# qfall/tools

Hardware: NVIDIA B200
Metric: samp_p_preimages_per_s (higher is better)
Workload: dtype f64

## Files before the change

### tools_b200/csrc/api.cu

```cuda
#include <algorithm>
#include <cmath>
#include <cstdio>
#include <cstring>
#include <string>
#include <vector>

#include "../../include/qfall_b200.h"
#include "common.cuh"
#include "kernels.h"

namespace {

typedef unsigned __int128 u128;
typedef __int128 i128;

struct Dev {
    void* p = nullptr;
    size_t cap = 0;
    cudaError_t ensure(size_t bytes) {
        if (bytes <= cap) return cudaSuccess;
        if (p) cudaFree(p);
        p = nullptr;
        cap = 0;
        cudaError_t e = cudaMalloc(&p, bytes);
// ... 715 lines not shown
        g.B = Bc; g.N = (int)ctx->m_bar; g.K = (int)ctx->nk;
        g.out_kind = 2; g.sign = 1; g.q = 0; g.base = nullptr; g.ldbase = 0; g.out = P; g.ldout = ldm;
        g.flag = ctx->dFlag.as<int>();
        LAUNCH(ctx_gemm_i8(ctx, g));
    } else {
        LAUNCH(ctx_gemm(ctx, Z, ldnk, ctx->dR.as<double>(), ldnk, P, ldm, Bc, (int)ctx->m_bar, (int)ctx->nk, 1.0, 1.0, 0));
    }
    LAUNCH(qf_launch_finalize_pert(P, ldm, Z, ldnk, dE, ctx->m, Bc, (int)ctx->m, (int)ctx->m_bar, ctx->dFlag.as<int>(),
                                   ctx->stream));
    return QF_OK;
}

qf_status samp_p_pert_chunk(qf_ctx* ctx, const int64_t* dUin, int Bc, uint64_t seed, uint64_t first, int32_t* dE,
                            const int32_t* dTidx = nullptr) {
    QF_TRY(pert_perturbation(ctx, Bc, seed, first));
    QF_TRY(pert_ap(ctx, dUin, Bc, ctx->w[4].as<int64_t>()));
    return pert_finish(ctx, Bc, seed, first, dE, dTidx);
}

constexpr long NP_SIZES[4] = {64, 256, 1024, 4096};
constexpr int NP_TOP = 4;
constexpr long NP_SCALE_BLOCK = NP_SIZES[3];
constexpr long NP_THIN = 512;
constexpr long NP_PROP_LD = NP_SIZES[2] + NP_THIN;

static long np_last_block_start(long D, long S) {
    long top = (D - 1) / S * S;
    if (top > 0 && D - top < NP_THIN) top -= S;
    return top;
}

qf_status gemm_i8_gated(qf_ctx* ctx, I8GemmArgs g, const int* gate, int lx_min = 3) {
    const int Lmax = g.LX;
    if (!gate || Lmax <= lx_min) {
        LAUNCH(ctx_gemm_i8(ctx, g));
        return QF_OK;
    }
    for (int lx = lx_min; lx <= Lmax; ++lx) {
        I8GemmArgs v = g;
        v.LX = lx;
        v.gate = gate;
        v.gate_lo = lx == lx_min ? 0 : lx - 1;
        v.gate_hi = lx == Lmax ? 1 << 20 : lx - 1;
        LAUNCH(ctx_gemm_i8(ctx, v, lx == Lmax));
    }
    return QF_OK;
}

static inline int np_block_index(long col, long D, long S) {
    return (int)(std::min(col, np_last_block_start(D, S)) / S);
}

qf_status np_block(qf_ctx* ctx, double* T, double* Z, int Bc, long lo, long hi, int level, long prop0, uint64_t seed,
                   uint64_t first) {
    const long D = ctx->dim, ldD = ctx->ld_dim;
    const double* U = ctx->dU.as<double>();
    if (level == 0) {
        NpDigitOut dig{};
        const bool fuse_digits = ctx->use_ozaki && ctx->np_fuse_split;
        if (fuse_digits && (lo & 63)) return ctx->fail(QF_ERR_NUMERIC, "internal: diagonal block not 64-aligned");
        if (fuse_digits) {
            const long ldk = ctx->ldk_dim;
            int* gates = ctx->dGate.as<int>();
            dig.planes = ctx->w[8].as<int8_t>(); dig.plane_stride = (long)ctx->chunk * ldk; dig.ldk = ldk; dig.L = ctx->z_limbs;
            dig.nz = ctx->dNz.as<uint8_t>(); dig.nz_m_tiles = (int)((ctx->chunk + 127) / 128); dig.nz_kb_total = (int)(ldk / 128);
            dig.gate[0] = gates + np_block_index(lo, D, NP_SIZES[1]);
            dig.gate[1] = gates + ctx->gate_n256 + np_block_index(lo, D, NP_SIZES[2]);
            dig.gate[2] = gates + ctx->gate_n256 + ctx->gate_n1024 + np_block_index(lo, D, NP_SIZES[3]);
            dig.gate[3] = (ctx->gpv_struct && hi > ctx->nk) ? gates + ctx->gate_n256 + ctx->gate_n1024 + ctx->gate_n4096 : nullptr;
        }
        LAUNCH(qf_launch_np_diag(T, ldD, Z, ldD, U, ldD, ctx->dDg.as<DGaussParams>(),
                                 ctx->w[9].as<float4>(), ctx->chunk, Bc, (int)lo, (int)(hi - lo), (int)D,
                                 seed, first, ctx->zlimit, ctx->dFlag.as<int>(), ctx->stream, (int)lo, fuse_digits ? &dig : nullptr,
                                 (int)prop0, ctx->np_diag_variant));
        return QF_OK;
    }
    if (level == 1 && ctx->np_fuse64 && (lo & 63) == 0)
        return np_block(ctx, T, Z, Bc, lo, hi, 0, prop0, seed, first);
    const long step = NP_SIZES[level - 1];
    const bool i8_level = level >= 2 && ctx->use_ozaki;
    for (long sub_hi = hi; sub_hi > lo;) {
        long sub_lo = std::max(lo, (sub_hi - 1) / step * step);
        if (i8_level && sub_hi == D && sub_lo > lo && sub_hi - sub_lo < NP_THIN) sub_lo = std::max(lo, sub_lo - step);
        if (level == 3) {
            CK(ctx->w[9].ensure((size_t)ctx->chunk * NP_PROP_LD * sizeof(float4)));
            LAUNCH(qf_launch_np_propose(ctx->w[9].as<float4>(), ctx->chunk, Bc, (int)sub_lo, (int)(sub_hi - sub_lo), (int)D,
                                        seed, first, ctx->stream));
            prop0 = sub_lo;
        }
        QF_TRY(np_block(ctx, T, Z, Bc, sub_lo, sub_hi, level - 1, prop0, seed, first));
        if (i8_level) {
            const long ldk = ctx->ldk_dim, plane = (long)ctx->chunk * ldk;
            const int nz_m = (int)((ctx->chunk + 127) / 128), nz_kb = (int)(ldk / 128);
            int8_t* zp = ctx->w[8].as<int8_t>();
            int* gates = ctx->dGate.as<int>();
            int* gate0 = gates + np_block_index(sub_lo, D, NP_SIZES[1]);
            int* gate1 = gates + ctx->gate_n256 + np_block_index(sub_lo, D, NP_SIZES[2]);
            int* gate4 = gates + ctx->gate_n256 + ctx->gate_n1024 + np_block_index(sub_lo, D, NP_SIZES[3]);
            int* gate_z2 = gates + ctx->gate_n256 + ctx->gate_n1024 + ctx->gate_n4096;
            if (level == 2 && !ctx->np_fuse_split)
                LAUNCH(qf_launch_split_f64_limbs(Z + sub_lo, ldD, zp + sub_lo, plane, ldk, Bc, (int)(sub_hi - sub_lo), ctx->z_limbs,
                                                 ctx->dFlag.as<int>(), ctx->dNz.as<uint8_t>(), nz_m, nz_kb, (int)sub_lo,
                                                 ctx->stream, gate0, gate1, gate4,
                                                 (ctx->gpv_struct && sub_hi > ctx->nk) ? gate_z2 : nullptr));
            if (sub_lo > lo && sub_hi - sub_lo < NP_SIZES[1]) {
                LAUNCH(ctx_gemm(ctx, Z + sub_lo, ldD, U + lo * ldD + sub_lo, ldD, T + lo, ldD, Bc, (int)(sub_lo - lo),
                                (int)(sub_hi - sub_lo), -1.0, 1.0, 0));
            } else if (sub_lo > lo) {
                I8GemmArgs g{};
                g.x = zp + sub_lo; g.ldx = ldk; g.x_plane = plane;
                const int wdrop = ctx->np_wdrop_cur;
                g.w = ctx->dUl.as<int8_t>() + (size_t)wdrop * D * ldk + lo * ldk + sub_lo; g.ldw = ldk; g.w_plane = D * ldk;
                g.LX = ctx->z_limbs; g.LW = ctx->u_limbs - wdrop; g.w_signed = 1;
// ... 56 lines not shown
        g.B = Bc; g.N = (int)D; g.K = np;
        g.out_kind = 3; g.sign = 1; g.q = 0; g.out = T; g.ldout = ldD;
        g.flag = ctx->dFlag.as<int>();
        g.scale = ctx->dMtPscale.as<double>();
        g.d_lo = ctx->np_dlo; g.overwrite = 1;
        LAUNCH(ctx_gemm_i8(ctx, g));
    } else {
        LAUNCH(ctx_gemm(ctx, Sol, ldp, ctx->dMtP.as<double>(), ldp, T, ldD, Bc, (int)D, np, -1.0, 0.0, 0));
    }
    if (ctx->use_ozaki) {
        const long ldk = ctx->ldk_dim;
        const size_t nzb = (size_t)ctx->z_limbs * ((ctx->chunk + 127) / 128) * (ldk / 128);
        CK(ctx->w[8].ensure((size_t)ctx->z_limbs * C * ldk));
        CK(ctx->dNz.ensure(nzb));
        CK(cudaMemsetAsync(ctx->dNz.p, 0, nzb, ctx->stream));
        ctx->gate_n256 = np_block_index(D - 1, D, NP_SIZES[1]) + 1;
        ctx->gate_n1024 = np_block_index(D - 1, D, NP_SIZES[2]) + 1;
        ctx->gate_n4096 = np_block_index(D - 1, D, NP_SIZES[3]) + 1;
        const size_t gb = (size_t)(ctx->gate_n256 + ctx->gate_n1024 + ctx->gate_n4096 + 1) * sizeof(int);
        CK(ctx->dGate.ensure(gb));
        CK(cudaMemsetAsync(ctx->dGate.p, 0, gb, ctx->stream));
    }
    ctx->np_wdrop_cur = 0; ctx->np_dlo_cur = ctx->np_dlo; ctx->np_lx_min = 3;
    QF_TRY(np_block(ctx, T, Z, Bc, 0, D, NP_TOP, 0, seed, first));
    if (ctx->use_i8) {
        const long ldk = ctx->ldk_dim, plane = C * ldk;
        int8_t* zp;
        I8GemmArgs g{};
        if (ctx->use_ozaki) {
            zp = ctx->w[8].as<int8_t>();
            g.x_nz = ctx->dNz.as<uint8_t>(); g.nz_m_tiles = (int)((ctx->chunk + 127) / 128); g.nz_kb_total = (int)(ldk / 128);
        } else {
            CK(ctx->w[2].ensure((size_t)std::max<long>(ctx->z_limbs * plane, C * ldD * 8)));
            zp = ctx->w[2].as<int8_t>();
            LAUNCH(qf_launch_split_f64_limbs(Z, ldD, zp, plane, ldk, Bc, (int)D, ctx->z_limbs, ctx->dFlag.as<int>(), nullptr, 0,
                                             0, 0, ctx->stream));
        }
        if (ctx->gpv_struct) {
            const long nk = ctx->nk, mb = ctx->m_bar, ldnk = ctx->ld_nk, ldk_nk = ctx->ldk_nk;
            CK(ctx->w[4].ensure((size_t)C * ldnk * 8));
            double* I2 = ctx->w[4].as<double>();
            CK(cudaMemsetAsync(I2, 0, (size_t)Bc * ldnk * 8, ctx->stream));
            g.x = zp + nk; g.ldx = ldk; g.x_plane = plane;
            g.w = ctx->dWl.p; g.ldw = ctx->ldk_mb; g.w_plane = nk * ctx->ldk_mb;
            g.LX = ctx->z_limbs; g.LW = 1; g.w_signed = 0;
            g.B = Bc; g.N = (int)nk; g.K = (int)mb;
            g.out_kind = 2; g.sign = 1; g.q = 0; g.base = nullptr; g.ldbase = 0; g.out = I2; g.ldout = ldnk;
// ... 67 lines not shown
    CK(ctx->w[0].ensure((size_t)C * n * 8));
    CK(ctx->w[2].ensure((size_t)C * ldD * 8));
    CK(ctx->w[3].ensure((size_t)C * ldD * 8));
    CK(ctx->w[4].ensure((size_t)C * ctx->ld_nk * 8));
    CK(ctx->w[8].ensure((size_t)L * plane));
    CK(ctx->w[10].ensure((size_t)C * ctx->ldk_nk));
    const size_t nzb = (size_t)L * nz_m * nz_kb;
    CK(ctx->dNz.ensure(nzb));
    CK(cudaMemsetAsync(ctx->dNz.p, 0, nzb, ctx->stream));
    ctx->gate_n256 = np_block_index(D - 1, D, NP_SIZES[1]) + 1;
    ctx->gate_n1024 = np_block_index(D - 1, D, NP_SIZES[2]) + 1;
    ctx->gate_n4096 = np_block_index(D - 1, D, NP_SIZES[3]) + 1;
    const size_t gb = (size_t)(ctx->gate_n256 + ctx->gate_n1024 + ctx->gate_n4096 + 1) * sizeof(int);
    CK(ctx->dGate.ensure(gb));
    CK(cudaMemsetAsync(ctx->dGate.p, 0, gb, ctx->stream));
    return QF_OK;
}

qf_status np2_phase1(qf_ctx* ctx, int Bc, uint64_t seed, uint64_t first) {
    const long D = ctx->dim, ldD = ctx->ld_dim, nk = ctx->nk;
    double* T = ctx->w[2].as<double>();
    CK(cudaMemset2DAsync(T + nk, (size_t)ldD * 8, 0, (size_t)ctx->m_bar * 8, (size_t)Bc, ctx->stream));
    ctx->np_wdrop_cur = ctx->u_limbs - ctx->u22_limbs; ctx->np_dlo_cur = ctx->u22_dlo; ctx->np_lx_min = 3;
    return np_block(ctx, T, ctx->w[3].as<double>(), Bc, nk, D, NP_TOP, 0, seed, first);
}

qf_status np2_abar_z2(qf_ctx* ctx, const int64_t* base, bool abar_tagged, int Bc, int64_t* out) {
    const long C = ctx->chunk, nk = ctx->nk, n = ctx->n, ldk = ctx->ldk_dim;
    const long ldw = abar_tagged ? ctx->ldk_mb : ldk;
    I8GemmArgs g{};
    g.x = ctx->w[8].as<int8_t>() + nk; g.ldx = ldk; g.x_plane = C * ldk;
    g.w = abar_tagged ? ctx->dAbpl.p : ctx->dAl.p; g.ldw = ldw; g.w_plane = n * ldw;
    g.LX = ctx->z_limbs; g.LW = ctx->a_limbs; g.w_signed = 0;
    g.B = Bc; g.N = (int)n; g.K = (int)ctx->m_bar;
    g.out_kind = 0; g.sign = -1; g.q = ctx->prm.q; g.base = base; g.ldbase = n;
    g.out = out; g.ldout = n;
    g.flag = ctx->dFlag.as<int>();
    g.x_nz = ctx->dNz.as<uint8_t>(); g.nz_m_tiles = (int)((C + 127) / 128); g.nz_kb_total = (int)(ldk / 128);
    g.nz_kb_off = (int)(nk / 128);
    return gemm_i8_gated(ctx, g, ctx->dGate.as<int>() + ctx->gate_n256 + ctx->gate_n1024 + ctx->gate_n4096);
}

qf_status np2_mt1_z2(qf_ctx* ctx, int Bc, double* out, long ldout, const double* scale, int overwrite) {
    const long C = ctx->chunk, nk = ctx->nk, ldk = ctx->ldk_dim;
    I8GemmArgs g{};
    g.x = ctx->w[8].as<int8_t>() + nk; g.ldx = ldk; g.x_plane = C * ldk;
    g.w = ctx->dMt1l.p; g.ldw = ctx->ldk_mb; g.w_plane = nk * ctx->ldk_mb;
// ... 18 lines not shown
    const bool fused_tail = (nk & 3) == 0 && (mb & 3) == 0 && (D & 3) == 0 && (ldk_nk & 3) == 0;
    double* I2 = ctx->w[4].as<double>();
    LAUNCH(qf_launch_gadget_digits(H, n, gp, ldk_nk, Bc, (int)n, (int)ctx->k, (unsigned)ctx->prm.base, nullptr, 0, ctx->stream,
                                   fused_tail ? nullptr : I2, ldnk));
    {
        I8GemmArgs g{};
        g.x = gp; g.ldx = ldk_nk; g.x_plane = C * ldk_nk;
        g.w = ctx->dMpl.p; g.ldw = ldk_nk; g.w_plane = nk * ldk_nk;
        g.LX = 1; g.LW = ctx->mt1g_limbs; g.w_signed = 1;
        g.B = Bc; g.N = (int)nk; g.K = (int)nk;
        g.out_kind = 3; g.sign = 1; g.q = 0; g.out = T; g.ldout = ldD;
        g.flag = flag;
        g.scale = ctx->dMpscale.as<double>();
        g.d_lo = 0; g.overwrite = 1;
        g.tri_mode = ctx->gpv_rev ? 3 : 4; g.tri_slack = (int)ctx->k;
        LAUNCH(ctx_gemm_i8(ctx, g));
    }
    if (Tpool)
        LAUNCH(qf_launch_pool_centre(Tpool, nk, T, ldD, ctx->dMt1scale.as<double>(), std::ldexp(1.0, 8 * ctx->mt1_dlo), (int)nk,
                                     Bc, ctx->stream));
    else
        QF_TRY(np2_mt1_z2(ctx, Bc, T, ldD, ctx->dMt1scale.as<double>(), 0));
    ctx->np_wdrop_cur = ctx->u_limbs - ctx->u11_limbs; ctx->np_dlo_cur = ctx->u11_dlo; ctx->np_lx_min = 2;
    QF_TRY(np_block(ctx, T, Z, Bc, 0, nk, NP_TOP, 0, seed, first));

    const long plane2 = C * ldk_nk;
    CK(ctx->w[2].ensure((size_t)std::max<long>(ctx->i2_limbs * plane2, C * ldD * 8)));
    int8_t* ip = ctx->w[2].as<int8_t>();
    if (fused_tail) {
        LAUNCH(qf_launch_gpv_ebot(Z, ldD, gp, ldk_nk, dE, D, (int)mb, ip, plane2, ldk_nk, ctx->i2_limbs, Bc, (int)nk, (int)ctx->k,
                                  ctx->dSkf.as<double>(), ctx->gpv_rev, flag, ctx->stream));
    } else {
        LAUNCH(qf_launch_sprime_apply(Z, ldD, I2, ldnk, Bc, (int)nk, (int)ctx->k, ctx->dSkf.as<double>(), ctx->gpv_rev,
                                      ctx->stream));
        LAUNCH(qf_launch_split_f64_limbs(I2, ldnk, ip, plane2, ldk_nk, Bc, (int)nk, ctx->i2_limbs, flag, nullptr, 0, 0, 0,
                                         ctx->stream));
    }
    {
        I8GemmArgs h{};
        h.x = ip; h.ldx = ldk_nk; h.x_plane = plane2;
        h.w = ctx->dRl.p; h.ldw = ldk_nk; h.w_plane = mb * ldk_nk;
        h.LX = ctx->i2_limbs; h.LW = 1; h.w_signed = 1;
        h.B = Bc; h.N = (int)mb; h.K = (int)nk;
        h.out_kind = 1; h.sign = 1; h.q = 0; h.out = dE; h.ldout = D;
        h.flag = flag;
        LAUNCH(ctx_gemm_i8(ctx, h));
    }
// ... 2983 lines not shown
```

### tools_b200/csrc/kernels.h

```cpp
#pragma once
#include <cuda_runtime.h>
#include <stdint.h>
#include "common.cuh"

cudaError_t qf_launch_gemm_f64(const double* X, long ldx, const double* W, long ldw, double* C, long ldc,
                               int B, int N, int K, double alpha, double beta, int tri_lower,
                               cudaStream_t stream);

cudaError_t qf_launch_i32_to_f64(const int32_t* in, long ldin, double* out, long ldout, int B, int M,
                                 unsigned long long* norm2, cudaStream_t stream);
cudaError_t qf_launch_i64_to_f64(const int64_t* in, long ldin, double* out, long ldout, int B, int M,
                                 double scale, cudaStream_t stream);
cudaError_t qf_launch_f64_to_i32(const double* in, long ldin, int32_t* out, long ldout, int B, int M,
                                 int* flag, cudaStream_t stream);
cudaError_t qf_launch_domain_flags(const unsigned long long* norm2, unsigned long long bound, uint8_t* flags,
                                   int B, cudaStream_t stream);

struct CombineArgs {
    const double* acc[4];
    int shift[4];
    int nacc;
    int acc_sign;
    long ldacc;
    const int64_t* base;
// ... 28 lines not shown
cudaError_t qf_launch_gadget_digits(const int64_t* h, long ldh, int8_t* plane, long ldk, int B, int n, int k, unsigned base,
                                    uint8_t* nz, int nz_kb_total, cudaStream_t stream, double* I2 = nullptr, long ldi = 0);
cudaError_t qf_launch_gadget_to_gso(const double* U, long ldu, int nk, int k, int rev, const double* skinv, double* out,
                                    long ldo, cudaStream_t stream);
cudaError_t qf_launch_pert_xb(const double* G, long ldg, double* X2, long ldx, int8_t* planes, long plane_stride, long ldk,
                              int B, int mb, int nk, double sqrt_beta, double fscale, int L, int* flag, cudaStream_t stream);
cudaError_t qf_launch_pert_normal_digits(int B, int M, int split, uint64_t seed, uint64_t first_target, int8_t* gplanes,
                                         long gplane_stride, long ldkg, int LG, double gscale, double* X2, long ldx,
                                         int8_t* bplanes, long bplane_stride, long ldkb, int LB, double sqrt_beta, double bscale,
                                         int* flag, cudaStream_t stream);
cudaError_t qf_launch_uniform_modq(int64_t* out, long count, unsigned long long q, uint64_t seed,
                                   uint64_t first_index, cudaStream_t stream);
cudaError_t qf_launch_ternary(int8_t* out, long count, uint64_t seed, cudaStream_t stream);

cudaError_t qf_launch_gadget_sample(const int64_t* V, long ldv, double* Z, long ldz, int B, int n, int k,
                                    int base, unsigned long long q, const double* sk, const double* gso,
                                    double s_g, uint64_t seed, uint64_t first_target, int* flag, cudaStream_t stream);
struct NpDigitOut {
    int8_t* planes; long plane_stride, ldk; int L;
    uint8_t* nz; int nz_m_tiles, nz_kb_total;
    int* gate[4];
};
cudaError_t qf_launch_np_diag(double* T, long ldt, double* Z, long ldz, const double* U, long ldu,
                              const DGaussParams* dg, const float4* prop, long ldprop, int B, int j0, int nb, int dim,
                              uint64_t seed, uint64_t first_target, double zlimit, int* flag, cudaStream_t stream, int up_lo = -1,
                              const NpDigitOut* dig = nullptr, int prop0 = -1, int variant = 0);
cudaError_t qf_launch_np_propose(float4* out, long ldo, int B, int j_lo, int width, int dim, uint64_t seed,
                                 uint64_t first_target, cudaStream_t stream);

cudaError_t qf_launch_compress_u16(const uint16_t* in, uint16_t* out, size_t count, uint32_t q, uint32_t d,
                                   int decompress, cudaStream_t stream);
cudaError_t qf_launch_byte_encode(const uint16_t* in, uint8_t* out, size_t npoly, uint32_t q, uint32_t d, int compress,
                                  cudaStream_t stream);
cudaError_t qf_launch_byte_decode(const uint8_t* in, uint16_t* out, size_t npoly, uint32_t q, uint32_t d, int decompress,
                                  cudaStream_t stream);
cudaError_t qf_launch_compress_i64(const int64_t* in, int64_t* out, size_t count, unsigned long long q,
                                   uint32_t d, int decompress, cudaStream_t stream);

cudaError_t qf_launch_encode_digits(const uint8_t* digits, void* coeffs, size_t count, unsigned long long q, unsigned base,
                                    int coeff_bytes, cudaStream_t stream);
cudaError_t qf_launch_decode_digits(const void* coeffs, uint8_t* digits, size_t count, unsigned long long q, unsigned base,
                                    int coeff_bytes, cudaStream_t stream);
cudaError_t qf_launch_encode_bits_u16(const uint8_t* msg, uint16_t* coeffs, size_t nbytes, uint32_t q, cudaStream_t stream);
cudaError_t qf_launch_decode_bits_u16(const uint16_t* coeffs, uint8_t* msg, size_t nbytes, uint32_t q, cudaStream_t stream);

void qf_ring_make_tables(int n, uint64_t* host_out);
cudaError_t qf_launch_ring_prepare(const int64_t* a, uint64_t* a_hat, long npoly, int n, unsigned long long q,
                                   const uint64_t* tw, cudaStream_t stream);
cudaError_t qf_launch_ring_f_a(const int32_t* sigma, const uint64_t* a_hat, int64_t* out, unsigned long long* norm2,
                               int B, int npoly, int n, unsigned long long q, const uint64_t* tw,
                               cudaStream_t stream, const int32_t* key_idx = nullptr, int nkeys = 0, int* flag = nullptr);
// ... 152 lines not shown
```

### tools_b200/csrc/lattice.cu

```cuda
#include <cstdlib>

#include "common.cuh"
#include "kernels.h"

namespace {

constexpr int GADGET_TPB = 128;
constexpr int KMAX = 64;

__global__ void __launch_bounds__(GADGET_TPB)
gadget_sample_kernel(const int64_t* __restrict__ V, long ldv, double* __restrict__ Z, long ldz, int B, int n, int k,
                     int base, unsigned long long q, const double* __restrict__ sk_g,
                     const double* __restrict__ gso_g, double s_g, uint64_t seed, uint64_t first_target, int* flag) {
    extern __shared__ __align__(16) double sm[];
    double* sk = sm;
    double* gs = sm + k * k;
    double* inv_n2 = gs + k * k;
    DGaussParams* dg = reinterpret_cast<DGaussParams*>(inv_n2 + k);
    for (int i = threadIdx.x; i < k * k; i += blockDim.x) {
        sk[i] = sk_g[i];
        gs[i] = gso_g[i];
    }
    __syncthreads();
    for (int i = threadIdx.x; i < k; i += blockDim.x) {
// ... 16 lines not shown
            v = (v - d) / (unsigned long long)base;
        }
        Philox rng;
        rng.init(seed, (first_target + (uint64_t)b) * (uint64_t)n + (uint64_t)row, QF_STREAM_GADGET);
        for (int i = k - 1; i >= 0; --i) {
            double dot = 0;
            for (int t = 0; t < k; ++t) dot += c[t] * gs[t * k + i];
            double z = sample_dgauss(dg[i], dot * inv_n2[i], rng, flag);
            if (z != 0.0)
                for (int t = 0; t < k; ++t) c[t] -= z * sk[t * k + i];
        }
        double* zr = Z + b * ldz + (long)row * k;
        for (int t = 0; t < k; ++t) zr[t] = -c[t];
    }
}

__device__ __noinline__ double np_sample_slow(DGaussParams dgp, double cp, uint64_t seed, uint64_t index, int* flag) {
    Philox ph;
    ph.init(seed, index, QF_STREAM_NP);
    ph.c3 = 1;
    return sample_dgauss(dgp, cp, ph, flag);
}

__global__ void __launch_bounds__(256)
np_propose_kernel(float4* __restrict__ out, long ldo, int B, int j_lo, int width, int dim, uint64_t seed,
                  uint64_t first_target) {
    const long total = (long)B * width;
    for (long idx = (long)blockIdx.x * blockDim.x + threadIdx.x; idx < total; idx += (long)gridDim.x * blockDim.x) {
        const int i = (int)(idx / B);
        const long b = idx - (long)i * B;
        Philox ph;
        ph.init(seed, (first_target + (uint64_t)b) * (uint64_t)dim + (uint64_t)(j_lo + i), QF_STREAM_NP);
        float n0, n1;
        ph.normal2(n0, n1);
        const float u0 = ph.uniform24(), u1 = ph.uniform24();
        out[(long)i * ldo + b] = make_float4(n0, n1, __logf(u0), __logf(u1));
    }
}

constexpr int NP_TPL = 2;
constexpr int NP_TARGETS = 32 * NP_TPL;
constexpr int NP_TPB = 128;
constexpr int NP_NB_MAX = 64;
constexpr int NP_TS = NP_NB_MAX + 1;
constexpr int NP_PANEL_LD = NP_NB_MAX + 2;
constexpr int NP_UST_DOUBLES = NP_NB_MAX * NP_PANEL_LD;

__global__ void __launch_bounds__(NP_TPB, 2)
np_diag_kernel(double* __restrict__ T, long ldt, double* __restrict__ Z, long ldz, const double* __restrict__ U,
               long ldu, const DGaussParams* __restrict__ dg_g, const float4* __restrict__ prop, long ldprop, int B,
               int j_lo, int j_hi, int prop0, int dim, uint64_t seed, uint64_t first_target, double zlimit, int* flag,
               int fuse_update, NpDigitOut dig) {
    extern __shared__ __align__(16) double np_sm[];
    double* ust = np_sm;
    double* ts = ust + NP_UST_DOUBLES;
    DGaussParams* dgs = reinterpret_cast<DGaussParams*>(ts + ((NP_TARGETS * NP_TS + 1) & ~1));
    const int tid = threadIdx.x, lane = tid & 31, warp = tid >> 5;
    const long b0 = (long)blockIdx.x * NP_TARGETS;
    const float4* const prop_base = prop;
    for (int sub_hi = j_hi; sub_hi > j_lo;) {
    const int j0 = max(j_lo, (sub_hi - 1) / NP_NB_MAX * NP_NB_MAX), nb = sub_hi - j0;
    const int up_lo = fuse_update ? j_lo : j0;
    const int us_ld = nb + 1;
    const int nbe = min(nb, dim - j0);
    prop = prop_base + (long)(j0 - prop0) * ldprop;
#pragma unroll 8
    for (int i = tid; i < nb * nb; i += NP_TPB) {
        const int r = i / nb, c = i - r * nb;
        ust[c * us_ld + r] = (r < nbe && c < nbe && c > r) ? U[(long)(j0 + r) * ldu + (j0 + c)] : 0.0;
    }
    for (int i = tid; i < nbe; i += NP_TPB) dgs[i] = dg_g[j0 + i];
#pragma unroll 4
    for (int r = warp; r < NP_TARGETS; r += NP_TPB / 32) {
        const long b = b0 + r;
        const double v0 = (b < B && lane < nbe) ? T[b * ldt + j0 + lane] : 0.0;
        const double v1 = (b < B && lane + 32 < nbe) ? T[b * ldt + j0 + lane + 32] : 0.0;
        ts[r * NP_TS + lane] = v0;
        ts[r * NP_TS + lane + 32] = v1;
    }
    __syncthreads();
    {
        const int tl = (tid >> 2) * NP_TPL, qd = tid & 3;
        const long bq = b0 + tl;
        constexpr int NG = NP_NB_MAX / 4;
        double c[NP_TPL][NG];
#pragma unroll
        for (int k = 0; k < NP_TPL; ++k)
#pragma unroll
            for (int j = 0; j < NG; ++j) c[k][j] = (4 * j + qd < nbe) ? ts[(tl + k) * NP_TS + 4 * j + qd] : 0.0;
        const float4* pq = prop + bq;
        float4 pcur[4][NP_TPL], pnxt[4][NP_TPL];
#pragma unroll
        for (int o = 0; o < 4; ++o) {
            const int ii = 4 * (NG - 1) + o;
#pragma unroll
            for (int k = 0; k < NP_TPL; ++k) pcur[o][k] = (ii < nbe) ? pq[(long)ii * ldprop + k] : make_float4(0.f, 0.f, 0.f, 0.f);
        }
        for (int kidx = 0; kidx < NG; ++kidx) {
            const int g = NG - 1 - kidx;
#pragma unroll
            for (int o = 0; o < 4; ++o) {
                const int in = 4 * (g - 1) + o;
#pragma unroll
                for (int k = 0; k < NP_TPL; ++k)
                    pnxt[o][k] = (g > 0 && in < nbe) ? pq[(long)in * ldprop + k] : make_float4(0.f, 0.f, 0.f, 0.f);
            }
#pragma unroll
            for (int owner = 3; owner >= 0; --owner) {
                const int ii = 4 * g + owner;
                if (ii < nbe) {
                    const DGaussParams dgp = dgs[ii];
                    double z[NP_TPL];
#pragma unroll
                    for (int k = 0; k < NP_TPL; ++k) {
                        const double cp = __shfl_sync(0xffffffffu, c[k][NG - 1], (lane & ~3) | owner);
                        const float4 pr = pcur[owner][k];
                        const double c_int = rint(cp);
                        const float c_frac = (float)(cp - c_int);
                        double zz = 0.0;
                        bool done = false;
                        {
                            float x = rintf(fmaf(dgp.sigma_p, pr.x, c_frac));
                            float d = x - c_frac;
                            float e = fmaf(-d * d, dgp.inv2s2, fmaf(0.5f * pr.x, pr.x, -dgp.emax));
                            if (fabsf(d) <= dgp.tail && pr.z < e) { zz = c_int + (double)x; done = true; }
                        }
                        if (!done) {
                            float x = rintf(fmaf(dgp.sigma_p, pr.y, c_frac));
                            float d = x - c_frac;
                            float e = fmaf(-d * d, dgp.inv2s2, fmaf(0.5f * pr.y, pr.y, -dgp.emax));
                            if (fabsf(d) <= dgp.tail && pr.w < e) { zz = c_int + (double)x; done = true; }
                        }
                        const bool live = bq + k < B;
                        if (!done && live)
                            zz = np_sample_slow(dgp, cp, seed, (first_target + (uint64_t)(bq + k)) * (uint64_t)dim + (uint64_t)(j0 + ii), flag);
                        if (live && qd == 0 && !(fabs(zz) < zlimit) && flag) atomicOr(flag, 2);
                        z[k] = zz;
                    }
                    const double* ucol = ust + ii * us_ld + qd;
                    {
                        const double u = ucol[4 * g];
#pragma unroll
                        for (int k = 0; k < NP_TPL; ++k) {
                            if (qd == owner) c[k][NG - 1] = z[k];
                            else if (qd < owner) c[k][NG - 1] = fma(-u, z[k], c[k][NG - 1]);
                        }
                    }
#pragma unroll
                    for (int kk = 0; kk < NG - 1; ++kk) {
                        const int grp = kk - kidx;
                        if (grp >= 0) {
                            const double u = ucol[4 * grp];
#pragma unroll
                            for (int k = 0; k < NP_TPL; ++k) c[k][kk] = fma(-u, z[k], c[k][kk]);
                        }
                    }
                }
            }
// ... 90 lines not shown
                }
            }
        }
    }
    __syncthreads();
    sub_hi = j0;
    }
}


constexpr int ND2_TPB = 128;
constexpr int ND2_LD = 72;
constexpr int ND2_ZLD = 136;
constexpr int ND2_PLD = 68;

__device__ __forceinline__ void nd2_dmma884(double& d0, double& d1, double a, double b) {
    asm volatile("mma.sync.aligned.m8n8k4.row.col.f64.f64.f64.f64 {%0,%1}, {%2}, {%3}, {%0,%1};\n"
                 : "+d"(d0), "+d"(d1)
                 : "d"(a), "d"(b));
}

__global__ void __launch_bounds__(ND2_TPB, 2)
np_diag2_kernel(double* __restrict__ T, long ldt, double* __restrict__ Z, long ldz, const double* __restrict__ U,
                long ldu, const DGaussParams* __restrict__ dg_g, const float4* __restrict__ prop, long ldprop, int B,
                int j_lo, int j_hi, int prop0, int dim, uint64_t seed, uint64_t first_target, double zlimit, int* flag,
                int fuse_update, NpDigitOut dig) {
    extern __shared__ __align__(16) double nd2_sm[];
    double* ur = nd2_sm;
    double* cs = ur + 64 * ND2_LD;
    DGaussParams* dgs = reinterpret_cast<DGaussParams*>(cs + 64 * ND2_ZLD);
    const int tid = threadIdx.x, lane = tid & 31;
    const long b0 = (long)blockIdx.x * ND2_TPB, b = b0 + tid;
    const bool live = b < B;
    double* const cst = cs + tid;
    bool tile_on_chip = false;
    for (int sub_hi = j_hi; sub_hi > j_lo;) {
        const int j0 = max(j_lo, (sub_hi - 1) / 64 * 64), nb = sub_hi - j0;
        const int up_lo = fuse_update ? j_lo : j0;
        const int nbe = min(nb, dim - j0);
        {
            const int mr = tid >> 6, mc = tid & 63;
            double mv[32];
#pragma unroll
            for (int r = 0; r < 32; ++r) {
                const int row = mr + 2 * r;
                mv[r] = (row < nbe && mc < nbe && mc > row) ? U[(long)(j0 + row) * ldu + (j0 + mc)] : 0.0;
            }
            __syncthreads();
#pragma unroll
            for (int r = 0; r < 32; ++r) ur[(mr + 2 * r) * ND2_LD + mc] = mv[r];
        }
        for (int i = tid; i < 64; i += ND2_TPB) dgs[i] = i < nbe ? dg_g[j0 + i] : DGaussParams{0.f, 0.f, 0.f, 0.f};
        const bool have_tile = tile_on_chip;
        tile_on_chip = false;
        if (!have_tile) {
            const double* tr = T + b * ldt + j0;
            if (live && nbe == 64 && ((((uintptr_t)tr) & 15) == 0)) {
#pragma unroll 8
                for (int i = 0; i < 32; ++i) {
                    const double2 v = reinterpret_cast<const double2*>(tr)[i];
                    cst[(2 * i) * ND2_ZLD] = v.x;
                    cst[(2 * i + 1) * ND2_ZLD] = v.y;
                }
            } else {
                for (int i = 0; i < 64; ++i) cst[i * ND2_ZLD] = (live && i < nbe) ? tr[i] : 0.0;
            }
        }
        const float4* pq = prop + (long)(j0 - prop0) * ldprop + b;
        const uint64_t index0 = (first_target + (uint64_t)b) * (uint64_t)dim + (uint64_t)j0;
        float4 pcur[8], pnxt[8];
#pragma unroll
        for (int t = 0; t < 8; ++t) pcur[t] = (live && 56 + t < nbe) ? pq[(long)(56 + t) * ldprop] : make_float4(0.f, 0.f, 0.f, 0.f);
        __syncthreads();
#pragma unroll 1
        for (int g = 7; g >= 0; --g) {
            const int ig = 8 * g;
#pragma unroll
            for (int t = 0; t < 8; ++t)
                pnxt[t] = (live && g > 0 && ig - 8 + t < nbe) ? pq[(long)(ig - 8 + t) * ldprop] : make_float4(0.f, 0.f, 0.f, 0.f);
            if (ig < nbe) {
                double c8[8], z8[8];
#pragma unroll
                for (int t = 0; t < 8; ++t) c8[t] = cst[(ig + t) * ND2_ZLD];
#pragma unroll
                for (int t = 7; t >= 0; --t) {
                    double zz = 0.0;
                    if (ig + t < nbe) {
                        const DGaussParams dgp = dgs[ig + t];
                        const float4 p4 = pcur[t];
                        const double cp = c8[t];
                        const double c_int = rint(cp);
                        const float c_frac = (float)(cp - c_int);
                        bool done = false;
                        {
                            float x = rintf(fmaf(dgp.sigma_p, p4.x, c_frac));
                            float d = x - c_frac;
                            float e = fmaf(-d * d, dgp.inv2s2, fmaf(0.5f * p4.x, p4.x, -dgp.emax));
                            if (fabsf(d) <= dgp.tail && p4.z < e) { zz = c_int + (double)x; done = true; }
                        }
                        if (!done) {
                            float x = rintf(fmaf(dgp.sigma_p, p4.y, c_frac));
                            float d = x - c_frac;
                            float e = fmaf(-d * d, dgp.inv2s2, fmaf(0.5f * p4.y, p4.y, -dgp.emax));
                            if (fabsf(d) <= dgp.tail && p4.w < e) { zz = c_int + (double)x; done = true; }
                        }
                        if (!done && live)
                            zz = np_sample_slow(dgp, cp, seed, index0 + (uint64_t)(ig + t), flag);
                        if (live && !(fabs(zz) < zlimit) && flag) atomicOr(flag, 2);
                        const double* ucol = ur + ig * ND2_LD + ig + t;
#pragma unroll
                        for (int tp = 0; tp < t; ++tp) c8[tp] = fma(-ucol[tp * ND2_LD], zz, c8[tp]);
                    }
                    z8[t] = zz;
                }
#pragma unroll
                for (int t = 0; t < 8; ++t) cst[(ig + t) * ND2_ZLD] = z8[t];
#pragma unroll 8
                for (int j = 0; j < ig; ++j) {
                    double cj = cst[j * ND2_ZLD];
                    const double2* up = reinterpret_cast<const double2*>(ur + j * ND2_LD + ig);
                    const double2 u01 = up[0], u23 = up[1], u45 = up[2], u67 = up[3];
                    cj = fma(-u67.y, z8[7], cj);
                    cj = fma(-u67.x, z8[6], cj);
                    cj = fma(-u45.y, z8[5], cj);
                    cj = fma(-u45.x, z8[4], cj);
                    cj = fma(-u23.y, z8[3], cj);
                    cj = fma(-u23.x, z8[2], cj);
                    cj = fma(-u01.y, z8[1], cj);
                    cj = fma(-u01.x, z8[0], cj);
                    cst[j * ND2_ZLD] = cj;
                }
            }
#pragma unroll
            for (int t = 0; t < 8; ++t) pcur[t] = pnxt[t];
        }
        double c[64];
#pragma unroll
        for (int i = 0; i < 64; ++i) c[i] = cst[i * ND2_ZLD];
        if (live) {
            double* zr = Z + b * ldz + j0;
            if (nbe == 64 && ((((uintptr_t)zr) & 15) == 0)) {
#pragma unroll
                for (int i = 0; i < 32; ++i) reinterpret_cast<double2*>(zr)[i] = make_double2(c[2 * i], c[2 * i + 1]);
            } else {
#pragma unroll
                for (int i = 0; i < 64; ++i)
                    if (i < nbe) zr[i] = c[i];
            }
        }
        if (dig.planes != nullptr) {
            int top = -1;
            long long bias = 0;
            for (int l = 0; l < dig.L; ++l) {
                int8_t* dst = dig.planes + (long)l * dig.plane_stride + b * dig.ldk + j0;
                unsigned any = 0;
                unsigned w[16];
                const bool last = l == dig.L - 1;
// ... 103 lines not shown
}

cudaError_t qf_launch_gadget_sample(const int64_t* V, long ldv, double* Z, long ldz, int B, int n, int k, int base,
                                    unsigned long long q, const double* sk, const double* gso, double s_g,
                                    uint64_t seed, uint64_t first_target, int* flag, cudaStream_t stream) {
    if (B <= 0) return cudaSuccess;
    if (k > KMAX) return cudaErrorInvalidValue;
    size_t smem = (size_t)(2 * k * k + k) * sizeof(double) + (size_t)k * sizeof(DGaussParams);
    static size_t configured_dev[QF_MAX_DEVICES] = {};
    size_t& configured = configured_dev[qf_device_slot()];
    if (smem > 48 * 1024 && smem > configured) {
        cudaError_t e = cudaFuncSetAttribute(gadget_sample_kernel, cudaFuncAttributeMaxDynamicSharedMemorySize, (int)smem);
        if (e != cudaSuccess) return e;
        configured = smem;
    }
    long long total = (long long)B * n;
    long long g = (total + GADGET_TPB - 1) / GADGET_TPB;
    if (g > 148 * 16) g = 148 * 16;
    gadget_sample_kernel<<<(int)g, GADGET_TPB, smem, stream>>>(V, ldv, Z, ldz, B, n, k, base, q, sk, gso, s_g, seed,
                                                               first_target, flag);
    return cudaGetLastError();
}

cudaError_t qf_launch_np_propose(float4* out, long ldo, int B, int j_lo, int width, int dim, uint64_t seed,
                                 uint64_t first_target, cudaStream_t stream) {
    if (B <= 0 || width <= 0) return cudaSuccess;
    long long total = (long long)B * width;
    long long g = (total + 255) / 256;
    if (g > 148 * 32) g = 148 * 32;
    np_propose_kernel<<<(int)g, 256, 0, stream>>>(out, ldo, B, j_lo, width, dim, seed, first_target);
    return cudaGetLastError();
}

cudaError_t qf_launch_np_diag(double* T, long ldt, double* Z, long ldz, const double* U, long ldu,
                              const DGaussParams* dg, const float4* prop, long ldprop, int B, int j0, int nb, int dim,
                              uint64_t seed, uint64_t first_target, double zlimit, int* flag, cudaStream_t stream, int up_lo,
                              const NpDigitOut* dig, int prop0, int variant) {
    if (B <= 0) return cudaSuccess;
    const bool multi = nb > NP_NB_MAX;
    if (nb < 1 || (multi && (up_lo != j0 || (j0 % NP_NB_MAX) != 0))) return cudaErrorInvalidValue;
    if (prop0 < 0) prop0 = j0;
    int grid = (B + NP_TARGETS - 1) / NP_TARGETS;
    if (up_lo < 0 || up_lo > j0) up_lo = j0;
    if ((up_lo < j0 || multi) && ((ldt & 1) || ((j0 - up_lo) & 15) || (up_lo & 1) || (((uintptr_t)T) & 15))) return cudaErrorInvalidValue;
    if (!multi && up_lo < j0) return cudaErrorInvalidValue;
    size_t smem = (size_t)(NP_UST_DOUBLES + ((NP_TARGETS * NP_TS + 1) & ~1)) * sizeof(double) +
                  (size_t)NP_NB_MAX * sizeof(DGaussParams);
    static size_t configured_dev[QF_MAX_DEVICES] = {};
    size_t& configured = configured_dev[qf_device_slot()];
    if (smem > 48 * 1024 && smem > configured) {
        cudaError_t e = cudaFuncSetAttribute(np_diag_kernel, cudaFuncAttributeMaxDynamicSharedMemorySize, (int)smem);
        if (e != cudaSuccess) return e;
        configured = smem;
    }
    NpDigitOut d{};
    if (dig) {
        d = *dig;
        if ((j0 & 63) || (d.ldk & 1) || (((uintptr_t)d.planes) & 1) || (d.plane_stride & 1)) return cudaErrorInvalidValue;
    }
    const bool v1 = variant == 1;
    const bool v2_ok = (!dig || (((d.ldk & 15) == 0) && ((((uintptr_t)d.planes) & 15) == 0) && ((d.plane_stride & 15) == 0))) &&
                       (ldt & 1) == 0 && ((((uintptr_t)T) & 15) == 0) && ((up_lo & 1) == 0);
    if (!v1 && v2_ok) {
        const size_t smem2 = (size_t)(64 * ND2_LD + 64 * ND2_ZLD) * sizeof(double) + 64 * sizeof(DGaussParams);
        static size_t configured2_dev[QF_MAX_DEVICES] = {};
        size_t& configured2 = configured2_dev[qf_device_slot()];
        if (smem2 > configured2) {
            cudaError_t e2 = cudaFuncSetAttribute(np_diag2_kernel, cudaFuncAttributeMaxDynamicSharedMemorySize, (int)smem2);
            if (e2 != cudaSuccess) return e2;
            configured2 = smem2;
        }
        np_diag2_kernel<<<(B + ND2_TPB - 1) / ND2_TPB, ND2_TPB, smem2, stream>>>(T, ldt, Z, ldz, U, ldu, dg, prop, ldprop, B, j0,
                                                                                 j0 + nb, prop0, dim, seed, first_target, zlimit,
                                                                                 flag, multi ? 1 : 0, d);
        return cudaGetLastError();
    }
    np_diag_kernel<<<grid, NP_TPB, smem, stream>>>(T, ldt, Z, ldz, U, ldu, dg, prop, ldprop, B, j0, j0 + nb, prop0, dim, seed,
                                                   first_target, zlimit, flag, multi ? 1 : 0, d);
    return cudaGetLastError();
}
```

Measured before the change: 615,300.

## Generate Gaussian proposals inline in diagonal kernels instead of separate propose pass

Removes the separate proposal kernel that wrote float4 Philox normals and log-uniforms to a global buffer, and instead computes them on the fly inside both diagonal sampling kernels. In the v2 kernel, the next group's proposals are generated interleaved with the first rows of the trailing update so the RNG latency can hide behind FMA work. This is meant to remove the global-memory write and read of the proposal buffer and one launch per level-3 block. In exchange, Philox work now sits on the sequential critical path and adds register pressure. An env-gated trace path with timing and fallback counters is also added.

```diff
diff --git a/tools_b200/csrc/api.cu b/tools_b200/csrc/api.cu
--- a/tools_b200/csrc/api.cu
+++ b/tools_b200/csrc/api.cu
@@ -761,7 +761,6 @@
 constexpr int NP_TOP = 4;
 constexpr long NP_SCALE_BLOCK = NP_SIZES[3];
 constexpr long NP_THIN = 512;
-constexpr long NP_PROP_LD = NP_SIZES[2] + NP_THIN;
 
 static long np_last_block_start(long D, long S) {
     long top = (D - 1) / S * S;
@@ -790,8 +789,7 @@
     return (int)(std::min(col, np_last_block_start(D, S)) / S);
 }
 
-qf_status np_block(qf_ctx* ctx, double* T, double* Z, int Bc, long lo, long hi, int level, long prop0, uint64_t seed,
-                   uint64_t first) {
+qf_status np_block(qf_ctx* ctx, double* T, double* Z, int Bc, long lo, long hi, int level, uint64_t seed, uint64_t first) {
     const long D = ctx->dim, ldD = ctx->ld_dim;
     const double* U = ctx->dU.as<double>();
     if (level == 0) {
@@ -808,26 +806,43 @@
             dig.gate[2] = gates + ctx->gate_n256 + ctx->gate_n1024 + np_block_index(lo, D, NP_SIZES[3]);
             dig.gate[3] = (ctx->gpv_struct && hi > ctx->nk) ? gates + ctx->gate_n256 + ctx->gate_n1024 + ctx->gate_n4096 : nullptr;
         }
-        LAUNCH(qf_launch_np_diag(T, ldD, Z, ldD, U, ldD, ctx->dDg.as<DGaussParams>(),
-                                 ctx->w[9].as<float4>(), ctx->chunk, Bc, (int)lo, (int)(hi - lo), (int)D,
-                                 seed, first, ctx->zlimit, ctx->dFlag.as<int>(), ctx->stream, (int)lo, fuse_digits ? &dig : nullptr,
-                                 (int)prop0, ctx->np_diag_variant));
+        auto launch = [&](unsigned long long* slow_cnt) {
+            return qf_launch_np_diag(T, ldD, Z, ldD, U, ldD, ctx->dDg.as<DGaussParams>(), Bc, (int)lo, (int)(hi - lo), (int)D,
+                                     seed, first, ctx->zlimit, ctx->dFlag.as<int>(), ctx->stream, (int)lo,
+                                     fuse_digits ? &dig : nullptr, ctx->np_diag_variant, slow_cnt);
+        };
+        static const bool trace = getenv("QF_TRACE") && getenv("QF_TRACE")[0] == '1';
+        if (trace) {
+            Dev cnt;
+            cudaEvent_t t0, t1;
+            CK(cnt.ensure(16));
+            CK(cudaMemsetAsync(cnt.p, 0, 16, ctx->stream));
+            CK(cudaEventCreate(&t0));
+            CK(cudaEventCreate(&t1));
+            CK(cudaEventRecord(t0, ctx->stream));
+            LAUNCH(launch(cnt.as<unsigned long long>()));
+            CK(cudaEventRecord(t1, ctx->stream));
+            CK(cudaStreamSynchronize(ctx->stream));
+            float ms = 0;
+            unsigned long long hh[2] = {0, 0};
+            CK(cudaEventElapsedTime(&ms, t0, t1));
+            CK(cudaMemcpy(hh, cnt.p, 16, cudaMemcpyDeviceToHost));
+            cudaEventDestroy(t0); cudaEventDestroy(t1);
+            fprintf(stderr, "[np_diag] B=%d lo=%ld hi=%ld nk=%ld %.3f ms  fallback: %llu of %lld warp-steps, %llu lanes\n", Bc, lo,
+                    hi, (long)ctx->nk, ms, hh[0], (long long)(Bc + 31) / 32 * (hi - lo), hh[1]);
+            return QF_OK;
+        }
+        LAUNCH(launch(nullptr));
         return QF_OK;
     }
     if (level == 1 && ctx->np_fuse64 && (lo & 63) == 0)
-        return np_block(ctx, T, Z, Bc, lo, hi, 0, prop0, seed, first);
+        return np_block(ctx, T, Z, Bc, lo, hi, 0, seed, first);
     const long step = NP_SIZES[level - 1];
     const bool i8_level = level >= 2 && ctx->use_ozaki;
     for (long sub_hi = hi; sub_hi > lo;) {
         long sub_lo = std::max(lo, (sub_hi - 1) / step * step);
         if (i8_level && sub_hi == D && sub_lo > lo && sub_hi - sub_lo < NP_THIN) sub_lo = std::max(lo, sub_lo - step);
-        if (level == 3) {
-            CK(ctx->w[9].ensure((size_t)ctx->chunk * NP_PROP_LD * sizeof(float4)));
-            LAUNCH(qf_launch_np_propose(ctx->w[9].as<float4>(), ctx->chunk, Bc, (int)sub_lo, (int)(sub_hi - sub_lo), (int)D,
-                                        seed, first, ctx->stream));
-            prop0 = sub_lo;
-        }
-        QF_TRY(np_block(ctx, T, Z, Bc, sub_lo, sub_hi, level - 1, prop0, seed, first));
+        QF_TRY(np_block(ctx, T, Z, Bc, sub_lo, sub_hi, level - 1, seed, first));
         if (i8_level) {
             const long ldk = ctx->ldk_dim, plane = (long)ctx->chunk * ldk;
             const int nz_m = (int)((ctx->chunk + 127) / 128), nz_kb = (int)(ldk / 128);
@@ -930,7 +945,7 @@
         CK(cudaMemsetAsync(ctx->dGate.p, 0, gb, ctx->stream));
     }
     ctx->np_wdrop_cur = 0; ctx->np_dlo_cur = ctx->np_dlo; ctx->np_lx_min = 3;
-    QF_TRY(np_block(ctx, T, Z, Bc, 0, D, NP_TOP, 0, seed, first));
+    QF_TRY(np_block(ctx, T, Z, Bc, 0, D, NP_TOP, seed, first));
     if (ctx->use_i8) {
         const long ldk = ctx->ldk_dim, plane = C * ldk;
         int8_t* zp;
@@ -1044,7 +1059,7 @@
     double* T = ctx->w[2].as<double>();
     CK(cudaMemset2DAsync(T + nk, (size_t)ldD * 8, 0, (size_t)ctx->m_bar * 8, (size_t)Bc, ctx->stream));
     ctx->np_wdrop_cur = ctx->u_limbs - ctx->u22_limbs; ctx->np_dlo_cur = ctx->u22_dlo; ctx->np_lx_min = 3;
-    return np_block(ctx, T, ctx->w[3].as<double>(), Bc, nk, D, NP_TOP, 0, seed, first);
+    return np_block(ctx, T, ctx->w[3].as<double>(), Bc, nk, D, NP_TOP, seed, first);
 }
 
 qf_status np2_abar_z2(qf_ctx* ctx, const int64_t* base, bool abar_tagged, int Bc, int64_t* out) {
@@ -1109,7 +1124,7 @@
     else
         QF_TRY(np2_mt1_z2(ctx, Bc, T, ldD, ctx->dMt1scale.as<double>(), 0));
     ctx->np_wdrop_cur = ctx->u_limbs - ctx->u11_limbs; ctx->np_dlo_cur = ctx->u11_dlo; ctx->np_lx_min = 2;
-    QF_TRY(np_block(ctx, T, Z, Bc, 0, nk, NP_TOP, 0, seed, first));
+    QF_TRY(np_block(ctx, T, Z, Bc, 0, nk, NP_TOP, seed, first));
 
     const long plane2 = C * ldk_nk;
     CK(ctx->w[2].ensure((size_t)std::max<long>(ctx->i2_limbs * plane2, C * ldD * 8)));
diff --git a/tools_b200/csrc/kernels.h b/tools_b200/csrc/kernels.h
--- a/tools_b200/csrc/kernels.h
+++ b/tools_b200/csrc/kernels.h
@@ -74,11 +74,9 @@
     int* gate[4];
 };
 cudaError_t qf_launch_np_diag(double* T, long ldt, double* Z, long ldz, const double* U, long ldu,
-                              const DGaussParams* dg, const float4* prop, long ldprop, int B, int j0, int nb, int dim,
-                              uint64_t seed, uint64_t first_target, double zlimit, int* flag, cudaStream_t stream, int up_lo = -1,
-                              const NpDigitOut* dig = nullptr, int prop0 = -1, int variant = 0);
-cudaError_t qf_launch_np_propose(float4* out, long ldo, int B, int j_lo, int width, int dim, uint64_t seed,
-                                 uint64_t first_target, cudaStream_t stream);
+                              const DGaussParams* dg, int B, int j0, int nb, int dim, uint64_t seed, uint64_t first_target,
+                              double zlimit, int* flag, cudaStream_t stream, int up_lo = -1, const NpDigitOut* dig = nullptr,
+                              int variant = 0, unsigned long long* slow_cnt = nullptr);
 
 cudaError_t qf_launch_compress_u16(const uint16_t* in, uint16_t* out, size_t count, uint32_t q, uint32_t d,
                                    int decompress, cudaStream_t stream);
diff --git a/tools_b200/csrc/lattice.cu b/tools_b200/csrc/lattice.cu
--- a/tools_b200/csrc/lattice.cu
+++ b/tools_b200/csrc/lattice.cu
@@ -62,20 +62,13 @@
     return sample_dgauss(dgp, cp, ph, flag);
 }
 
-__global__ void __launch_bounds__(256)
-np_propose_kernel(float4* __restrict__ out, long ldo, int B, int j_lo, int width, int dim, uint64_t seed,
-                  uint64_t first_target) {
-    const long total = (long)B * width;
-    for (long idx = (long)blockIdx.x * blockDim.x + threadIdx.x; idx < total; idx += (long)gridDim.x * blockDim.x) {
-        const int i = (int)(idx / B);
-        const long b = idx - (long)i * B;
-        Philox ph;
-        ph.init(seed, (first_target + (uint64_t)b) * (uint64_t)dim + (uint64_t)(j_lo + i), QF_STREAM_NP);
-        float n0, n1;
-        ph.normal2(n0, n1);
-        const float u0 = ph.uniform24(), u1 = ph.uniform24();
-        out[(long)i * ldo + b] = make_float4(n0, n1, __logf(u0), __logf(u1));
-    }
+__device__ __forceinline__ float4 np_proposal(uint64_t seed, uint64_t index) {
+    Philox ph;
+    ph.init(seed, index, QF_STREAM_NP);
+    float n0, n1;
+    ph.normal2(n0, n1);
+    const float u0 = ph.uniform24(), u1 = ph.uniform24();
+    return make_float4(n0, n1, __logf(u0), __logf(u1));
 }
 
 constexpr int NP_TPL = 2;
@@ -88,22 +81,19 @@
 
 __global__ void __launch_bounds__(NP_TPB, 2)
 np_diag_kernel(double* __restrict__ T, long ldt, double* __restrict__ Z, long ldz, const double* __restrict__ U,
-               long ldu, const DGaussParams* __restrict__ dg_g, const float4* __restrict__ prop, long ldprop, int B,
-               int j_lo, int j_hi, int prop0, int dim, uint64_t seed, uint64_t first_target, double zlimit, int* flag,
-               int fuse_update, NpDigitOut dig) {
+               long ldu, const DGaussParams* __restrict__ dg_g, int B, int j_lo, int j_hi, int dim, uint64_t seed,
+               uint64_t first_target, double zlimit, int* flag, int fuse_update, NpDigitOut dig) {
     extern __shared__ __align__(16) double np_sm[];
     double* ust = np_sm;
     double* ts = ust + NP_UST_DOUBLES;
     DGaussParams* dgs = reinterpret_cast<DGaussParams*>(ts + ((NP_TARGETS * NP_TS + 1) & ~1));
     const int tid = threadIdx.x, lane = tid & 31, warp = tid >> 5;
     const long b0 = (long)blockIdx.x * NP_TARGETS;
-    const float4* const prop_base = prop;
     for (int sub_hi = j_hi; sub_hi > j_lo;) {
     const int j0 = max(j_lo, (sub_hi - 1) / NP_NB_MAX * NP_NB_MAX), nb = sub_hi - j0;
     const int up_lo = fuse_update ? j_lo : j0;
     const int us_ld = nb + 1;
     const int nbe = min(nb, dim - j0);
-    prop = prop_base + (long)(j0 - prop0) * ldprop;
 #pragma unroll 8
     for (int i = tid; i < nb * nb; i += NP_TPB) {
         const int r = i / nb, c = i - r * nb;
@@ -128,13 +118,15 @@
         for (int k = 0; k < NP_TPL; ++k)
 #pragma unroll
             for (int j = 0; j < NG; ++j) c[k][j] = (4 * j + qd < nbe) ? ts[(tl + k) * NP_TS + 4 * j + qd] : 0.0;
-        const float4* pq = prop + bq;
+        uint64_t index0[NP_TPL];
+#pragma unroll
+        for (int k = 0; k < NP_TPL; ++k) index0[k] = (first_target + (uint64_t)(bq + k)) * (uint64_t)dim + (uint64_t)j0;
         float4 pcur[4][NP_TPL], pnxt[4][NP_TPL];
 #pragma unroll
         for (int o = 0; o < 4; ++o) {
             const int ii = 4 * (NG - 1) + o;
 #pragma unroll
-            for (int k = 0; k < NP_TPL; ++k) pcur[o][k] = (ii < nbe) ? pq[(long)ii * ldprop + k] : make_float4(0.f, 0.f, 0.f, 0.f);
+            for (int k = 0; k < NP_TPL; ++k) pcur[o][k] = (ii < nbe) ? np_proposal(seed, index0[k] + ii) : make_float4(0.f, 0.f, 0.f, 0.f);
         }
         for (int kidx = 0; kidx < NG; ++kidx) {
             const int g = NG - 1 - kidx;
@@ -143,7 +135,7 @@
                 const int in = 4 * (g - 1) + o;
 #pragma unroll
                 for (int k = 0; k < NP_TPL; ++k)
-                    pnxt[o][k] = (g > 0 && in < nbe) ? pq[(long)in * ldprop + k] : make_float4(0.f, 0.f, 0.f, 0.f);
+                    pnxt[o][k] = (g > 0 && in < nbe) ? np_proposal(seed, index0[k] + in) : make_float4(0.f, 0.f, 0.f, 0.f);
             }
 #pragma unroll
             for (int owner = 3; owner >= 0; --owner) {
@@ -173,7 +165,7 @@
                         }
                         const bool live = bq + k < B;
                         if (!done && live)
-                            zz = np_sample_slow(dgp, cp, seed, (first_target + (uint64_t)(bq + k)) * (uint64_t)dim + (uint64_t)(j0 + ii), flag);
+                            zz = np_sample_slow(dgp, cp, seed, index0[k] + ii, flag);
                         if (live && qd == 0 && !(fabs(zz) < zlimit) && flag) atomicOr(flag, 2);
                         z[k] = zz;
                     }
@@ -310,9 +302,9 @@
 
 __global__ void __launch_bounds__(ND2_TPB, 2)
 np_diag2_kernel(double* __restrict__ T, long ldt, double* __restrict__ Z, long ldz, const double* __restrict__ U,
-                long ldu, const DGaussParams* __restrict__ dg_g, const float4* __restrict__ prop, long ldprop, int B,
-                int j_lo, int j_hi, int prop0, int dim, uint64_t seed, uint64_t first_target, double zlimit, int* flag,
-                int fuse_update, NpDigitOut dig) {
+                long ldu, const DGaussParams* __restrict__ dg_g, int B, int j_lo, int j_hi, int dim, uint64_t seed,
+                uint64_t first_target, double zlimit, int* flag, int fuse_update, NpDigitOut dig,
+                unsigned long long* slow_cnt) {
     extern __shared__ __align__(16) double nd2_sm[];
     double* ur = nd2_sm;
     double* cs = ur + 64 * ND2_LD;
@@ -326,6 +318,8 @@
         const int j0 = max(j_lo, (sub_hi - 1) / 64 * 64), nb = sub_hi - j0;
         const int up_lo = fuse_update ? j_lo : j0;
         const int nbe = min(nb, dim - j0);
+        const uint64_t index0 = (first_target + (uint64_t)b) * (uint64_t)dim + (uint64_t)j0;
+        float4 prop[8];
         {
             const int mr = tid >> 6, mc = tid & 63;
             double mv[32];
@@ -334,6 +328,8 @@
                 const int row = mr + 2 * r;
                 mv[r] = (row < nbe && mc < nbe && mc > row) ? U[(long)(j0 + row) * ldu + (j0 + mc)] : 0.0;
             }
+#pragma unroll
+            for (int t = 0; t < 8; ++t) prop[t] = np_proposal(seed, index0 + (uint64_t)(56 + t));
             __syncthreads();
 #pragma unroll
             for (int r = 0; r < 32; ++r) ur[(mr + 2 * r) * ND2_LD + mc] = mv[r];
@@ -354,19 +350,11 @@
                 for (int i = 0; i < 64; ++i) cst[i * ND2_ZLD] = (live && i < nbe) ? tr[i] : 0.0;
             }
         }
-        const float4* pq = prop + (long)(j0 - prop0) * ldprop + b;
-        const uint64_t index0 = (first_target + (uint64_t)b) * (uint64_t)dim + (uint64_t)j0;
-        float4 pcur[8], pnxt[8];
-#pragma unroll
-        for (int t = 0; t < 8; ++t) pcur[t] = (live && 56 + t < nbe) ? pq[(long)(56 + t) * ldprop] : make_float4(0.f, 0.f, 0.f, 0.f);
         __syncthreads();
 #pragma unroll 1
         for (int g = 7; g >= 0; --g) {
             const int ig = 8 * g;
-#pragma unroll
-            for (int t = 0; t < 8; ++t)
-                pnxt[t] = (live && g > 0 && ig - 8 + t < nbe) ? pq[(long)(ig - 8 + t) * ldprop] : make_float4(0.f, 0.f, 0.f, 0.f);
-            if (ig < nbe) {
+            {
                 double c8[8], z8[8];
 #pragma unroll
                 for (int t = 0; t < 8; ++t) c8[t] = cst[(ig + t) * ND2_ZLD];
@@ -375,7 +363,7 @@
                     double zz = 0.0;
                     if (ig + t < nbe) {
                         const DGaussParams dgp = dgs[ig + t];
-                        const float4 p4 = pcur[t];
+                        const float4 p4 = prop[t];
                         const double cp = c8[t];
                         const double c_int = rint(cp);
                         const float c_frac = (float)(cp - c_int);
@@ -392,6 +380,13 @@
                             float e = fmaf(-d * d, dgp.inv2s2, fmaf(0.5f * p4.y, p4.y, -dgp.emax));
                             if (fabsf(d) <= dgp.tail && p4.w < e) { zz = c_int + (double)x; done = true; }
                         }
+                        if (slow_cnt) {
+                            const unsigned m = __ballot_sync(0xffffffffu, !done && live);
+                            if (m && lane == 0) {
+                                atomicAdd(slow_cnt, 1ull);
+                                atomicAdd(slow_cnt + 1, (unsigned long long)__popc(m));
+                            }
+                        }
                         if (!done && live)
                             zz = np_sample_slow(dgp, cp, seed, index0 + (uint64_t)(ig + t), flag);
                         if (live && !(fabs(zz) < zlimit) && flag) atomicOr(flag, 2);
@@ -403,8 +398,7 @@
                 }
 #pragma unroll
                 for (int t = 0; t < 8; ++t) cst[(ig + t) * ND2_ZLD] = z8[t];
-#pragma unroll 8
-                for (int j = 0; j < ig; ++j) {
+                auto update_row = [&](int j) {
                     double cj = cst[j * ND2_ZLD];
                     const double2* up = reinterpret_cast<const double2*>(ur + j * ND2_LD + ig);
                     const double2 u01 = up[0], u23 = up[1], u45 = up[2], u67 = up[3];
@@ -417,10 +411,17 @@
                     cj = fma(-u01.y, z8[1], cj);
                     cj = fma(-u01.x, z8[0], cj);
                     cst[j * ND2_ZLD] = cj;
-                }
-            }
-#pragma unroll
-            for (int t = 0; t < 8; ++t) pcur[t] = pnxt[t];
+                };
+                if (g > 0) {
+#pragma unroll
+                    for (int t = 0; t < 8; ++t) {
+                        prop[t] = np_proposal(seed, index0 + (uint64_t)(ig - 8 + t));
+                        update_row(t);
+                    }
+                }
+#pragma unroll 8
+                for (int j = 8; j < ig; ++j) update_row(j);
+            }
         }
         double c[64];
 #pragma unroll
@@ -570,24 +571,13 @@
     return cudaGetLastError();
 }
 
-cudaError_t qf_launch_np_propose(float4* out, long ldo, int B, int j_lo, int width, int dim, uint64_t seed,
-                                 uint64_t first_target, cudaStream_t stream) {
-    if (B <= 0 || width <= 0) return cudaSuccess;
-    long long total = (long long)B * width;
-    long long g = (total + 255) / 256;
-    if (g > 148 * 32) g = 148 * 32;
-    np_propose_kernel<<<(int)g, 256, 0, stream>>>(out, ldo, B, j_lo, width, dim, seed, first_target);
-    return cudaGetLastError();
-}
-
 cudaError_t qf_launch_np_diag(double* T, long ldt, double* Z, long ldz, const double* U, long ldu,
-                              const DGaussParams* dg, const float4* prop, long ldprop, int B, int j0, int nb, int dim,
-                              uint64_t seed, uint64_t first_target, double zlimit, int* flag, cudaStream_t stream, int up_lo,
-                              const NpDigitOut* dig, int prop0, int variant) {
+                              const DGaussParams* dg, int B, int j0, int nb, int dim, uint64_t seed, uint64_t first_target,
+                              double zlimit, int* flag, cudaStream_t stream, int up_lo, const NpDigitOut* dig, int variant,
+                              unsigned long long* slow_cnt) {
     if (B <= 0) return cudaSuccess;
     const bool multi = nb > NP_NB_MAX;
     if (nb < 1 || (multi && (up_lo != j0 || (j0 % NP_NB_MAX) != 0))) return cudaErrorInvalidValue;
-    if (prop0 < 0) prop0 = j0;
     int grid = (B + NP_TARGETS - 1) / NP_TARGETS;
     if (up_lo < 0 || up_lo > j0) up_lo = j0;
     if ((up_lo < j0 || multi) && ((ldt & 1) || ((j0 - up_lo) & 15) || (up_lo & 1) || (((uintptr_t)T) & 15))) return cudaErrorInvalidValue;
@@ -618,12 +608,12 @@
             if (e2 != cudaSuccess) return e2;
             configured2 = smem2;
         }
-        np_diag2_kernel<<<(B + ND2_TPB - 1) / ND2_TPB, ND2_TPB, smem2, stream>>>(T, ldt, Z, ldz, U, ldu, dg, prop, ldprop, B, j0,
-                                                                                 j0 + nb, prop0, dim, seed, first_target, zlimit,
-                                                                                 flag, multi ? 1 : 0, d);
+        np_diag2_kernel<<<(B + ND2_TPB - 1) / ND2_TPB, ND2_TPB, smem2, stream>>>(T, ldt, Z, ldz, U, ldu, dg, B, j0, j0 + nb, dim,
+                                                                                 seed, first_target, zlimit, flag, multi ? 1 : 0,
+                                                                                 d, slow_cnt);
         return cudaGetLastError();
     }
-    np_diag_kernel<<<grid, NP_TPB, smem, stream>>>(T, ldt, Z, ldz, U, ldu, dg, prop, ldprop, B, j0, j0 + nb, prop0, dim, seed,
-                                                   first_target, zlimit, flag, multi ? 1 : 0, d);
+    np_diag_kernel<<<grid, NP_TPB, smem, stream>>>(T, ldt, Z, ldz, U, ldu, dg, B, j0, j0 + nb, dim, seed, first_target, zlimit,
+                                                   flag, multi ? 1 : 0, d);
     return cudaGetLastError();
 }
```

After: 616,600, median of 6. No clear change (+0.2%).
